# ChenKaiXuSan/Skiing_Analysis_PyTorch

Measured on AMD Instinct MI355X. Metric: 3D-pose frames/sec, 8-view 518px clips, higher is better.
Workload: dtype f16

## Files before the change

### include/skimi.h

```cpp
#ifndef SKIMI_H
#define SKIMI_H

#include <stddef.h>
#include <stdint.h>

#ifdef __cplusplus
extern "C" {
#endif

#define SKIMI_OK 0
#define SKIMI_ERR_ARG (-1)
#define SKIMI_ERR_HIP (-2)
#define SKIMI_ERR_STATE (-3)
#define SKIMI_ERR_WORKSPACE (-4)

#define SKIMI_F32 0
#define SKIMI_BF16 1
#define SKIMI_BF16X3_REC 2
#define SKIMI_FP8MX 3
#define SKIMI_F16 4

#define SKIMI_PREC_BF16 0
#define SKIMI_PREC_BF16X3 1
#define SKIMI_PREC_FP8 2
// ... 47 lines not shown
    int32_t force_splitk;
    int32_t splitk_scratch_zeroed;
    const void* W_split;
    void* x3_scratch;
    uint64_t x3_scratch_bytes;
    void* out_records;
} skimi_gemm_desc;

int skimi_split_planes(const float* x, int64_t ld, int64_t rows, int32_t C, void* hi, void* lo, void* stream);

int skimi_split_records(const float* x, int64_t ld, int64_t rows, int32_t C, void* records, void* stream);

int skimi_dpt_fold_pack(const float* w_T, const float* b_T, const float* w_rn, int32_t C_in, int32_t C_mid, int32_t C_out,
                        int32_t s, void* w_records, float* beta, void* stream);

int skimi_gemm(const skimi_gemm_desc* d, void* stream);

#define SKIMI_GEMM_PATH_GENERIC 1
#define SKIMI_GEMM_PATH_SPLITK_ORDERED 2
#define SKIMI_GEMM_PATH_SPLITK_ATOMIC 3
#define SKIMI_GEMM_PATH_X3DMA_WIDE 4
#define SKIMI_GEMM_PATH_X3DMA_NARROW 5
#define SKIMI_GEMM_PATH_GEMM256 6
#define SKIMI_GEMM_PATH_CONV_WIN 7
int32_t skimi_gemm_last_path(void);

int skimi_quant_mx(const void* x, int32_t dtype, int64_t ldx, int64_t rows, int32_t K, void* payload, void* scales,
                   void* stream);
int skimi_layernorm_mx(const float* x, int64_t ldx, int64_t rows, int32_t C, const float* gamma, const float* beta,
                       float eps, void* payload, void* scales, void* stream);
// ... 90 lines not shown
    float* pose_enc;
    float* pose_enc_list;
    float* depth;
    float* depth_conf;
    float* world_points;
    float* world_points_conf;
    float* track;
    float* vis;
    float* conf;
    float* tokens_last;
} skimi_vggt_outputs;

int skimi_vggt_forward(skimi_vggt*, const float* images, const float* query_points, int32_t B, int32_t S,
                       int32_t H, int32_t W, int32_t n_query, const skimi_vggt_outputs* out,
                       void* workspace, size_t workspace_bytes, void* stream);

int skimi_pose_to_cameras(const float* pose_enc, int64_t rows, int32_t H, int32_t W, float* extrinsic,
                          float* intrinsic, void* stream);
int skimi_unproject_depth(const float* depth, const float* extrinsic, const float* intrinsic,
                          float* world_points, int32_t frames, int32_t H, int32_t W, void* stream);
int skimi_triangulate_dlt(const float* K, const float* R, const float* t, const float* keypoints,
                          float* joints3d, int64_t steps, int32_t views, int32_t joints, void* stream);

int skimi_triangulate_triage(const float* K, const float* R, const float* t, const float* keypoints, const float* conf,
                             double conf_thr, double err_thresh_px, int64_t steps, int32_t views, int32_t joints,
                             float* joints3d, float* joints3d_clean, double* err, double* depth, uint8_t* keep,
                             double* view_stats, double* report, void* stream);

int skimi_triangulate_robust(const float* K, const float* R, const float* t, const float* keypoints, const float* conf,
                             double conf_thr, double inlier_px, int32_t min_inliers, int32_t refine_iters, int32_t weighted,
// ... 319 lines not shown
```

### skiing_analysis_pytorch_amd/_lib.py

```python
from __future__ import annotations

import ctypes as C
from pathlib import Path

LIB_PATH = Path(__file__).resolve().parent / "lib" / "libskimi.so"

F32, BF16 = 0, 1
F16 = 4
BF16X3_REC = 2
FP8MX = 3
PREC_BF16, PREC_BF16X3, PREC_FP8 = 0, 1, 2
PREC_F16 = 3
ACT_NONE, ACT_RELU, ACT_GELU, ACT_SILU, ACT_SIGMOID = 0, 1, 2, 3, 4
GEMM_PATH_GENERIC, GEMM_PATH_SPLITK_ORDERED, GEMM_PATH_SPLITK_ATOMIC = 1, 2, 3
GEMM_PATH_X3DMA_WIDE, GEMM_PATH_X3DMA_NARROW, GEMM_PATH_GEMM256, GEMM_PATH_CONV_WIN = 4, 5, 6, 7
VP3D_CONV, VP3D_MM, VP3D_WIN, VP3D_EXPAND_MFMA, VP3D_EXPAND_VALU = 1, 2, 3, 4, 5


class SkimiError(RuntimeError):
    pass


class GemmDesc(C.Structure):

# ... 220 lines not shown
    "skimi_track_pos_embed_sample": (C.c_int, [_vp, C.c_int64, _vp, C.c_int32, C.c_int32, C.c_int32, C.c_int32, _vp]),
    "skimi_track_input": (C.c_int, [_vp, _vp, _vp, _vp, _vp, _vp, C.c_int64, C.c_int32, C.c_int32, C.c_int64, C.c_float, _vp]),
    "skimi_track_coord_update": (C.c_int, [_vp, _vp, C.c_int64, _vp, _vp, C.c_int64, C.c_int32, C.c_int32, C.c_float, _vp]),
    "skimi_track_init": (C.c_int, [_vp, _vp, _vp, C.c_int64, C.c_int32, C.c_float, _vp]),
    "skimi_track_repeat_rows": (C.c_int, [_vp, _vp, C.c_int64, C.c_int32, C.c_int32, _vp]),
    "skimi_track_bns_to_bsn": (C.c_int, [_vp, _vp, C.c_int32, C.c_int32, C.c_int32, _vp]),
    "skimi_vggt_create": (_vp, [_vp]),
    "skimi_vggt_destroy": (None, [_vp]),
    "skimi_vggt_set_weight": (C.c_int, [_vp, C.c_char_p, _vp, C.c_int64, C.c_int32]),
    "skimi_vggt_finalize": (C.c_int, [_vp]),
    "skimi_vggt_set_pos_embed": (C.c_int, [_vp, C.c_int32, C.c_int32, _vp, C.c_int32]),
    "skimi_vggt_rope_positions": (C.c_int, [_vp, C.c_int32, C.c_int32, C.c_int32, _vp]),
    "skimi_vggt_workspace_bytes": (C.c_size_t, [_vp, C.c_int32, C.c_int32, C.c_int32, C.c_int32, C.c_int32]),
    "skimi_vggt_forward": (C.c_int, [_vp, _vp, _vp, C.c_int32, C.c_int32, C.c_int32, C.c_int32, C.c_int32, _vp,
                                     _vp, C.c_size_t, _vp]),
}

_lib = None


def exported_symbols():
    return sorted(_SIGNATURES)


def lib() -> C.CDLL:
    global _lib
    if _lib is not None:
        return _lib
    if not LIB_PATH.exists():
        raise SkimiError(
# ... 37 lines not shown
```

### skiing_analysis_pytorch_amd/csrc/api.hip

```cpp
#include <stdarg.h>

#include <mutex>
#include <vector>

#include "common.h"
#include "gemm_epilogue.h"
#include "kernels.h"
#include "track_kernels.h"
#include "vggt_kernels.h"

namespace skimi {

static thread_local char g_err[512] = "";

void set_error(const char* fmt, ...) {
    va_list ap;
    va_start(ap, fmt);
    vsnprintf(g_err, sizeof(g_err), fmt, ap);
    va_end(ap);
}

int lds_opt_in(std::atomic<unsigned>& done, const void* kernel, int bytes, const char* what) {
    int dev = 0;
    if (hipGetDevice(&dev) != hipSuccess) {
// ... 157 lines not shown
    return split_records_launch(x, (long)ld, (long)rows, C, records, (hipStream_t)stream);
}

int skimi_dpt_fold_pack(const float* w_T, const float* b_T, const float* w_rn, int32_t C_in, int32_t C_mid, int32_t C_out,
                        int32_t s, void* w_records, float* beta, void* stream) {
    SKIMI_CHECK_ARG(w_T && w_rn && w_records && beta, "skimi_dpt_fold_pack: null buffer");
    SKIMI_CHECK_ARG(s >= 2 && s <= 16 && C_in > 0 && C_in % 32 == 0 && C_mid > 0 && C_out > 0, "skimi_dpt_fold_pack: bad sizes");
    float* tmp = nullptr;
    SKIMI_HIP(hipMalloc((void**)&tmp, (size_t)(s + 2) * (s + 2) * C_out * C_in * 4));
    const int rc = dpt_fold_pack_launch(w_T, b_T, w_rn, C_in, C_mid, C_out, s, tmp, w_records, beta, (hipStream_t)stream);
    const hipError_t e = hipStreamSynchronize((hipStream_t)stream);
    (void)hipFree(tmp);
    if (rc) return rc;
    SKIMI_HIP(e);
    return SKIMI_OK;
}

int skimi_quant_mx(const void* x, int32_t dtype, int64_t ldx, int64_t rows, int32_t K, void* payload, void* scales,
                   void* stream) {
    return quant_mx_launch(x, dtype, (long)ldx, (long)rows, K, payload, scales, (hipStream_t)stream);
}

int skimi_layernorm_mx(const float* x, int64_t ldx, int64_t rows, int32_t C, const float* gamma, const float* beta,
                       float eps, void* payload, void* scales, void* stream) {
    return layernorm_mx_launch(x, ldx, rows, C, gamma, beta, eps, payload, scales, (hipStream_t)stream);
}

int skimi_gemm_fp8(const void* A, const void* A_scales, const void* W, const void* W_scales, int32_t M, int32_t N,
                   int32_t K, const float* bias, int32_t act, const float* gamma, const float* resid, int64_t ldr,
                   void* out, int32_t out_dtype, int64_t ldo, void* out_scales, void* stream) {
// ... 264 lines not shown
```

### skiing_analysis_pytorch_amd/csrc/vggt.hip

```cpp
#include <math.h>
#include <stdlib.h>
#include <string.h>

#include <map>
#include <memory>
#include <mutex>
#include <vector>

#include "kernels.h"
#include "vggt_kernels.h"
#include "vggt_model.h"

using namespace skimi;
using namespace skimi::vggt;

static int prepare(skimi_vggt* h, int F, int S, int H, int W, const ShapeTabs** out) {
    auto& entries = h->tabs[std::make_pair(H, W)];
    int largest = 0;
    for (const auto& e : entries) {
        if (e->frames >= F) {
            *out = e.get();
            return SKIMI_OK;
        }
        largest = std::max(largest, e->frames);
// ... 178 lines not shown
        }
    if (run_depth) {
        float* pts = out->depth ? out->depth : (float*)c.ar.alloc((size_t)F * H * W * 4);
        float* cf = out->depth_conf ? out->depth_conf : (float*)c.ar.alloc((size_t)F * H * W * 4);
        run_dpt(c, h->depth, sf, sg, F, P, nsp, ph, pw, C, H, W, pts, cf, 0);
    }
    if (run_point) {
        float* pts = out->world_points ? out->world_points : (float*)c.ar.alloc((size_t)F * H * W * 3 * 4);
        float* cf = out->world_points_conf ? out->world_points_conf : (float*)c.ar.alloc((size_t)F * H * W * 4);
        run_dpt(c, h->point, sf, sg, F, P, nsp, ph, pw, C, H, W, pts, cf, 1);
    }
    if (do_track) run_track(c, sf, sg, B, S, P, nsp, ph, pw, C, H, W, query, nq, out->track, out->vis, out->conf);
    return c.rc;
}

extern "C" {

skimi_vggt* skimi_vggt_create(const skimi_vggt_config* cfg) {
    if (!cfg) { set_error("skimi_vggt_create: null config"); return nullptr; }
    if (cfg->embed_dim <= 0 || cfg->num_heads <= 0 || cfg->embed_dim / cfg->num_heads != 64 ||
        cfg->embed_dim % cfg->num_heads != 0) {
        set_error("skimi_vggt_create: embed_dim / num_heads must be 64");
        return nullptr;
    }
    if (cfg->use_dino && cfg->embed_dim / cfg->dino_heads != 64) {
        set_error("skimi_vggt_create: DINOv2 head_dim must be 64");
        return nullptr;
    }
    if (cfg->patch_size <= 0 || cfg->depth <= 0 || cfg->num_register_tokens < 0) {
        set_error("skimi_vggt_create: bad sizes");
// ... 4 lines not shown
            set_error("skimi_vggt_create: dpt_layers[%d] = %d outside [0, depth)", i, cfg->dpt_layers[i]);
            return nullptr;
        }
    if (cfg->prec < SKIMI_PREC_BF16 || cfg->prec > SKIMI_PREC_F16) {
        set_error("skimi_vggt_create: prec %d is not one of SKIMI_PREC_BF16 / BF16X3 / FP8 / F16", cfg->prec);
        return nullptr;
    }
    if (cfg->head_prec != SKIMI_PREC_BF16 && cfg->head_prec != SKIMI_PREC_BF16X3 && cfg->head_prec != SKIMI_PREC_F16) {
        set_error("skimi_vggt_create: head_prec %d: the depth / point heads run in SKIMI_PREC_BF16X3 (the reference's fp32) or, as a "
                  "faster, less accurate option, on SKIMI_PREC_F16 / SKIMI_PREC_BF16 operands", cfg->head_prec);
        return nullptr;
    }
    skimi_vggt* h = new skimi_vggt();
    h->cfg = *cfg;
    h->dpt_fold = !(getenv("SKIMI_DPT_FOLD") && atoi(getenv("SKIMI_DPT_FOLD")) == 0);
    return h;
}

void skimi_vggt_destroy(skimi_vggt* h) {
    if (!h) return;
    for (auto& kv : h->raw) (void)hipFree(kv.second.first);
    for (void* p : h->owned) (void)hipFree(p);
    h->tabs.clear();
    for (auto& kv : h->dino_pos_alt) (void)hipFree(kv.second);
    delete h;
}

int skimi_vggt_set_weight(skimi_vggt* h, const char* key, const float* data, int64_t n, int32_t on_device) {
    SKIMI_CHECK_ARG(h && key && data && n > 0, "skimi_vggt_set_weight: bad arguments");
    float* d = nullptr;
// ... 112 lines not shown
        std::lock_guard<std::mutex> lk(h->prep_mu);
        if ((rc = prepare(h, B * S, S, H, W, &tabs))) return rc;
    }
    Ctx c{h, (hipStream_t)stream};
    c.tabs = tabs;
    c.ar.base = (char*)workspace;
    c.ar.cap = workspace_bytes;
    {
        Ctx dry{h, nullptr};
        dry.ar.dry = true;
        forward_impl(h, dry, images, query_points, B, S, H, W, n_query, out);
        if (dry.ar.peak > workspace_bytes) {
            set_error("skimi_vggt_forward: workspace %zu < %zu", workspace_bytes, dry.ar.peak);
            return SKIMI_ERR_WORKSPACE;
        }
    }
    return forward_impl(h, c, images, query_points, B, S, H, W, n_query, out);
}

}
```

### skiing_analysis_pytorch_amd/csrc/vggt_dpt.hip

```cpp
#include "env.h"
#include "gemm_epilogue.h"
#include "kernels.h"
#include "vggt_kernels.h"
#include "vggt_model.h"

namespace skimi {
namespace vggt {

const UvTab* find_uv(const ShapeTabs* h, int w, int hh, int C) {
    if (!h) return nullptr;
    for (const auto& t : h->uv)
        if (t.w == w && t.h == hh && t.C == C) return &t;
    return nullptr;
}

bool dpt_fused_ln(const DptW& w, int f2, int udt) {
    const bool off = !(int)env_once("SKIMI_TRACK_LN_FUSED", 1);
    return !off && w.feature_only && w.out_ln != nullptr && w.out_ln->g != nullptr && w.out_ln->b != nullptr && f2 == 128 && udt == SKIMI_F32;
}

static int uv_missing() {
    set_error("uv table missing");
    return SKIMI_ERR_STATE;
}

void* run_dpt(Ctx& c, const DptW& w, float* const* sf, float* const* sg, int F, int P, int nsp, int ph, int pw, int C,
              int H, int W, float* pts, float* conf, int act_mode) {
    const int prec = w.proj[0].prec;
    const int adt = Ctx::act_dt(prec);
    const size_t es = Ctx::esz(adt);
    const int D = 2 * C, np = ph * pw, feat = w.features;
    const size_t mk = c.ar.mark();
    int hh[4] = {ph * 4, ph * 2, ph, (ph - 1) / 2 + 1};
    int ww[4] = {pw * 4, pw * 2, pw, (pw - 1) / 2 + 1};
// ... 73 lines not shown
                c.gemm(d);
            }
            {
                auto d = c.desc(w.rn[i].lin, t1, adt, w.oc[i], F * hh[i] * ww[i], rn[i], adt, feat);
                c.conv_geom(d, w.rn[i], F, hh[i], ww[i], hh[i], ww[i]);
                d.act = SKIMI_ACT_RELU;
                d.out_records = rn_rec[i];
                c.gemm(d);
            }
            c.ar.release(mk3);
        }
        c.ar.release(mk2);
    }
    void* prev = nullptr;
    char* prev_rec = nullptr;
    for (int r = 3; r >= 0; --r) {
        const FusionW& f = w.ref[r];
        const int h0 = hh[r], w0 = ww[r];
        const int M = F * h0 * w0;
        const size_t bytes = (size_t)M * feat * es;
        const bool recs = use_rec[r];
        auto conv_in = [&](const ConvW& cw, const void* in_f32, char* in_rec, void* out_f32, char* out_rec) {
            auto d = c.desc(cw.lin, in_f32, adt, feat, M, out_f32, adt, feat);
            c.conv_geom(d, cw, F, h0, w0, h0, w0);
            if (recs) d = Ctx::as_records(d, in_rec, rec_bytes(r) - 256);
            d.out_records = out_rec;
            return d;
        };
        void* cur;
        char* cur_rec = nullptr;
// ... 14 lines not shown
            cur = rn[r];
            cur_rec = rn_rec[r];
        }
        const bool u_recs = recs && takes_records(f.out_conv, nullptr, r);
        void* u = u_recs ? nullptr : c.ar.alloc(bytes);
        char* u_rec = u_recs ? (char*)c.ar.alloc(rec_bytes(r)) : nullptr;
        {
            auto d1 = conv_in(f.r2c1, cur, cur_rec, tmp, tmp_rec);
            d1.act = SKIMI_ACT_RELU;
            c.gemm(d1);
            auto d2 = conv_in(f.r2c2, tmp, tmp_rec, u, u_rec);
            d2.resid = cur; d2.ldr = feat; d2.resid_dtype = adt;
            c.gemm(d2);
        }
        const int h1 = r > 0 ? hh[r - 1] : 2 * h0, w1 = r > 0 ? ww[r - 1] : 2 * w0;
        void* olow = c.ar.alloc(bytes);
        {
            auto d = c.desc(f.out_conv, u, adt, feat, M, olow, adt, feat);
            if (u_recs) d = Ctx::as_records(d, u_rec, rec_bytes(r) - 256);
            c.gemm(d);
        }
        if (r == 0 && adt == SKIMI_F32 && w.oc1.lin.w_split != nullptr && feat % 32 == 0) {
            const size_t rec_bytes = (size_t)F * h1 * w1 * feat * 4;
            const size_t mk_rec = c.ar.mark();
            char* rec = (char*)c.ar.alloc(rec_bytes + 256);
            auto d = Ctx::as_records(c.desc(w.oc1.lin, nullptr, adt, feat, F * h1 * w1, rec, adt, w.feature_only ? feat : feat / 2), rec,
                                     rec_bytes);
            c.conv_geom(d, w.oc1, F, h1, w1, h1, w1);
            if (gemm_x3dma_eligible(&d)) {
                prev_rec = rec;
// ... 2 lines not shown
                                                     nullptr, nullptr, 1, rec + rec_bytes);
                });
                prev = nullptr;
                hh[r] = h1; ww[r] = w1;
                continue;
            }
            c.ar.release(mk_rec);
        }
        void* o = c.ar.alloc((size_t)F * h1 * w1 * feat * es);
        c.run([&] { return bilinear_ac_launch(olow, o, adt, F, h0, w0, h1, w1, feat, c.st); });
        prev = o;
        hh[r] = h1; ww[r] = w1;
    }
    const int h1 = hh[0], w1 = ww[0];
    const int f2 = w.feature_only ? feat : feat / 2;
    void* c1 = c.ar.alloc((size_t)F * h1 * w1 * f2 * es);
    if (prev_rec != nullptr) {
        auto d = Ctx::as_records(c.desc(w.oc1.lin, nullptr, adt, feat, F * h1 * w1, c1, adt, f2), prev_rec, (size_t)F * h1 * w1 * feat * 4);
        c.conv_geom(d, w.oc1, F, h1, w1, h1, w1);
        c.gemm(d);
    } else {
        auto d = c.desc(w.oc1.lin, prev, adt, feat, F * h1 * w1, c1, adt, f2);
        c.conv_geom(d, w.oc1, F, h1, w1, h1, w1);
        c.gemm(d);
    }
    const int Ho = ph * c.h->cfg.patch_size / w.down_ratio, Wo = pw * c.h->cfg.patch_size / w.down_ratio;
    const UvTab* uvt = w.pos_embed ? find_uv(c.tabs, Wo, Ho, f2) : nullptr;
    if (w.pos_embed && !uvt) c.run(uv_missing);
    const int no_direct = !(int)env_once("SKIMI_CONV_DIRECT", 1);
    const bool direct = !w.feature_only && w.oc2a_direct != nullptr && adt == SKIMI_F32 && !no_direct;
    void* c2 = nullptr;
    if (direct) {
// ... 44 lines not shown
```

### skiing_analysis_pytorch_amd/csrc/vggt_kernels.h

```cpp
#pragma once
#include "common.h"

namespace skimi {

int patch_gather_launch(const float* img, void* out, int out_dtype, int F, int H, int W, int p, int Kp,
                        hipStream_t st);
int special_tokens_launch(float* x, const float* table, int F, int S, int P, int n, int C, hipStream_t st);
int bilinear_ac_planes_launch(const float* in, unsigned short* out, int N, int h, int w, int H, int W, int C, hipStream_t st,
                              const float* tabx = nullptr, const float* taby = nullptr,
                              int slice_records = 0, void* zpage = nullptr);
int bilinear_ac_launch(const void* in, void* out, int dtype, int N, int h, int w, int H, int W, int C,
                       hipStream_t st, const float* tabx = nullptr, const float* taby = nullptr, int out_dtype = -1,
                       const float* ln_g = nullptr, const float* ln_b = nullptr, float ln_eps = 0.f);
int add_uv_pos_launch(void* x, int dtype, const float* tabx, const float* taby, int N, int H, int W, int C,
                      hipStream_t st);
int add_uv_pos_records_launch(const float* x, const float* tabx, const float* taby, int N, int H, int W, int C, void* rec,
                              hipStream_t st);
int dpt_fold_pack_launch(const float* wT, const float* bT, const float* wrn, int Ci, int Cm, int Co, int s, float* tmp, void* rec,
                         float* beta, hipStream_t st);
int adaln_launch(const float* xn, const float* x, const float* mod, float* out, long rows, int D, hipStream_t st);
int pose_update_launch(const float* delta, float* pred_pad, float* act_out, long rows, int first, hipStream_t st);
int dpt_out_launch(const void* in, int dtype, const float* W, const float* b, int n_out, float* pts, float* conf,
                   long npix, int mode, hipStream_t st);
int f32_to_bf16_launch(const float* in, void* out, long n, hipStream_t st);
int f32_to_f16_launch(const float* in, void* out, long n, hipStream_t st);
int permute_conv_launch(const float* in, float* out, int Co, int Ci, int kh, int kw, hipStream_t st, int slice_major = 0);
int permute_convT_launch(const float* in, float* out, int Ci, int Co, int s, hipStream_t st);
int pad_cols_launch(const float* in, float* out, long rows, int K, int Kp, hipStream_t st);
int tile_vec_launch(const float* in, float* out, int n, int reps, hipStream_t st);

struct BilinearTap {
    int i0, i1;
    float l0, l1;
};
// ... 24 lines not shown
```

### skiing_analysis_pytorch_amd/csrc/vggt_kernels.hip

```cpp
#include <algorithm>

#include "common.h"
#include "gemm_epilogue.h"
#include "vggt_kernels.h"

namespace skimi {

static inline int grid_for(long n, int per_block = 256, int cap = 8192) {
    return (int)std::max<long>(1, std::min<long>(cdiv(n, per_block), cap));
}

template <typename T, bool F16 = false>
__global__ __launch_bounds__(256) void patch_gather_kernel(const float* __restrict__ img, T* __restrict__ out,
                                                           int F, int H, int W, int p, int Kp) {
    const int ph = H / p, pw = W / p, K = 3 * p * p;
    const long total = (long)F * ph * pw * Kp;
    const float mean[3] = {0.485f, 0.456f, 0.406f};
    const float stdv[3] = {0.229f, 0.224f, 0.225f};
    for (long i = (long)blockIdx.x * 256 + threadIdx.x; i < total; i += (long)gridDim.x * 256) {
        const int k = (int)(i % Kp);
        const long r = i / Kp;
        float v = 0.f;
        if (k < K) {
            const int px = (int)(r % pw);
// ... 391 lines not shown
            x = (int)((i / Ci) % kw);
            y = (int)((i / ((long)Ci * kw)) % kh);
            co = i / ((long)Ci * kw * kh);
        }
        out[i] = in[((co * Ci + ci) * kh + y) * kw + x];
    }
}
int permute_conv_launch(const float* in, float* out, int Co, int Ci, int kh, int kw, hipStream_t st, int slice_major) {
    SKIMI_CHECK_ARG(!slice_major || Ci % 32 == 0, "slice-major conv weights need Cin %% 32 == 0");
    hipLaunchKernelGGL(permute_conv_kernel, dim3(grid_for((long)Co * Ci * kh * kw)), dim3(256), 0, st, in, out, Co, Ci, kh, kw,
                       slice_major);
    SKIMI_LAUNCH_CHECK();
    return SKIMI_OK;
}

__global__ void permute_convT_kernel(const float* __restrict__ in, float* __restrict__ out, int Ci, int Co, int s) {
    const long n = (long)Ci * Co * s * s;
    for (long i = (long)blockIdx.x * 256 + threadIdx.x; i < n; i += (long)gridDim.x * 256) {
        const int ci = (int)(i % Ci);
        const long r = i / Ci;
        const int co = (int)(r % Co);
        const int ab = (int)(r / Co);
        const int a = ab / s, b = ab - a * s;
        out[i] = in[(((long)ci * Co + co) * s + a) * s + b];
    }
}
int permute_convT_launch(const float* in, float* out, int Ci, int Co, int s, hipStream_t st) {
    hipLaunchKernelGGL(permute_convT_kernel, dim3(grid_for((long)Ci * Co * s * s)), dim3(256), 0, st, in, out, Ci, Co, s);
    SKIMI_LAUNCH_CHECK();
    return SKIMI_OK;
// ... 125 lines not shown
```

### skiing_analysis_pytorch_amd/csrc/vggt_model.h

```cpp
#pragma once
#include <string.h>

#include <map>
#include <memory>
#include <mutex>
#include <string>
#include <utility>
#include <vector>

#include "common.h"

namespace skimi {
namespace vggt {

struct Lin {
    void* w = nullptr;
    int wdt = SKIMI_F32;
    float* b = nullptr;
    int N = 0, K = 0;
    int prec = SKIMI_PREC_BF16X3;
    void* w_split = nullptr;
    void* wq = nullptr;
    void* wq_scales = nullptr;
};
// ... 3 lines not shown
    Lin qkv, proj, fc1, fc2;
    float *ls1 = nullptr, *ls2 = nullptr;
    float *qn_w = nullptr, *qn_b = nullptr, *kn_w = nullptr, *kn_b = nullptr;
};
struct ConvW { Lin lin; int k = 1, stride = 1, pad = 0, cin = 0; int kmode = 1; };
struct FusionW { Lin out_conv; ConvW r1c1, r1c2, r2c1, r2c2; bool has_r1 = false; };
struct DptW {
    LNw norm;
    Lin proj[4];
    Lin rs0, rs1;
    Lin fold[2];
    ConvW rs3;
    ConvW rn[4];
    FusionW ref[4];
    ConvW oc1, oc2a;
    float *oc2b_w = nullptr, *oc2b_b = nullptr;
    unsigned short* oc2a_direct = nullptr;
    int n_out = 0, features = 0, oc[4] = {0, 0, 0, 0};
    bool feature_only = false, pos_embed = true;
    bool out_f32 = false;
    const LNw* out_ln = nullptr;
    int down_ratio = 1;
};
struct CamW {
    std::vector<BlockW> trunk;
    LNw token_norm, trunk_norm;
    float* empty16 = nullptr;
    Lin embed_pose, poseLN, fc1, fc2;
};
struct MhaW {
// ... 38 lines not shown
    std::vector<UvTab> uv;
    std::vector<void*> owned;
    ~ShapeTabs() {
        for (void* p : owned) (void)hipFree(p);
    }
};

}
}

struct skimi_vggt {
    skimi_vggt_config cfg;
    std::map<std::string, std::pair<float*, int64_t>> raw;
    std::vector<void*> owned;
    bool finalized = false;
    bool dpt_fold = true;
    skimi::vggt::Lin patch_proj;
    int patch_kp = 0;
    float* dino_pos = nullptr;
    std::map<std::pair<int, int>, float*> dino_pos_alt;
    float* dino_special = nullptr;
    float* agg_special = nullptr;
    std::vector<skimi::vggt::BlockW> dino, frame, global;
    skimi::vggt::LNw dino_norm;
    skimi::vggt::CamW cam;
    skimi::vggt::DptW depth, point, trackf;
    skimi::vggt::TrackW track;
    std::mutex prep_mu;
    std::map<std::pair<int, int>, std::vector<std::unique_ptr<skimi::vggt::ShapeTabs>>> tabs;
};
// ... 4 lines not shown
struct Packer {
    skimi_vggt* h;
    int rc = SKIMI_OK;
    hipStream_t st = nullptr;

    float* raw(const std::string& key, int64_t n);
    void* dmalloc(size_t bytes);
    float* keep(const std::string& key, int64_t n);
    LNw ln(const std::string& p, int C) { return LNw{keep(p + ".weight", C), keep(p + ".bias", C)}; }
    Lin pack_matrix(float* src, int N, int K, int prec);
    Lin linear(const std::string& p, int N, int K, int prec, bool bias = true);
    Lin linear_named(const std::string& wkey, const std::string& bkey, int N, int K, int prec);
    void add_records(Lin& L);
    ConvW conv(const std::string& p, int Co, int Ci, int k, int stride, int pad, int prec, bool bias);
    Lin convT(const std::string& p, int C, int s, int prec);
    Lin conv_fold(const std::string& pT, const std::string& pRn, int C, int Co, int s);
    void add_fp8(Lin& L, const std::string& p, int N, int K);
    BlockW block(const std::string& p, int C, int hidden, bool qk_norm, int hd, int prec_in);
    DptW dpt(const std::string& p, int D, int features, const int* oc, int n_out, bool feature_only, int prec);
};

int pack_model(skimi_vggt* h);
void pack_track(Packer& pk, skimi_vggt* h);

struct Ctx {
    skimi_vggt* h;
    hipStream_t st;
    const ShapeTabs* tabs = nullptr;
    Arena ar;
    int rc = SKIMI_OK;
// ... 20 lines not shown
    void ln(const float* x, const float* x2, long ldx, long rows, int C, const LNw& w, float eps, void* out, int odt,
            long grp_rows = 0, long grp_stride = 0, long grp_off = 0);
    void copy(void* dst, const void* src, size_t bytes);
    void zero(void* dst, size_t bytes);
};

struct BlockBufs { void* xn; void* qkv; void* ao; void* hid; void* q8 = nullptr; void* q8s = nullptr; };
struct MhaBufs { float *xn, *cn, *q, *kv, *ao, *hid; };

void run_block(Ctx& c, const BlockW& w, float* x, int batch, int seq, int C, int heads, float eps, bool rope,
               const BlockBufs& b);
void run_camera(Ctx& c, const CamW& w, const float* sf, const float* sg, int B, int S, int P, int C, float* out_list,
                float* out_last);
const UvTab* find_uv(const ShapeTabs* h, int w, int hh, int C);
bool dpt_fused_ln(const DptW& w, int f2, int udt);
void* run_dpt(Ctx& c, const DptW& w, float* const* sf, float* const* sg, int F, int P, int nsp, int ph, int pw, int C,
              int H, int W, float* pts, float* conf, int act_mode);
void run_track(Ctx& c, float* const* sf, float* const* sg, int B, int S, int P, int nsp, int ph, int pw, int C, int H, int W,
               const float* query, int N, float* out_track, float* out_vis, float* out_conf);

}
}
```

### skiing_analysis_pytorch_amd/csrc/vggt_pack.hip

```cpp
#include <stdlib.h>

#include "env.h"
#include "gemm_epilogue.h"
#include "kernels.h"
#include "vggt_kernels.h"
#include "vggt_model.h"

namespace skimi {
namespace vggt {

float* Packer::raw(const std::string& key, int64_t n) {
    if (rc) return nullptr;
    auto it = h->raw.find(key);
    if (it == h->raw.end()) {
        set_error("skimi_vggt_finalize: missing weight '%s'", key.c_str());
        rc = SKIMI_ERR_STATE;
        return nullptr;
    }
    if (it->second.second != n) {
        set_error("skimi_vggt_finalize: weight '%s' has %ld elements, expected %ld", key.c_str(),
                  (long)it->second.second, (long)n);
        rc = SKIMI_ERR_STATE;
        return nullptr;
    }
// ... 83 lines not shown
}
Lin Packer::convT(const std::string& p, int C, int s, int prec) {
    Lin L;
    float* src = raw(p + ".weight", (int64_t)C * C * s * s);
    float* bsrc = raw(p + ".bias", C);
    if (rc) return L;
    float* tmp = nullptr;
    if (hipMalloc((void**)&tmp, (size_t)C * C * s * s * 4) != hipSuccess) { rc = SKIMI_ERR_HIP; return L; }
    if ((rc = permute_convT_launch(src, tmp, C, C, s, st))) return L;
    L = pack_matrix(tmp, s * s * C, C, prec);
    if (!rc && prec == SKIMI_PREC_BF16X3 && C % 32 == 0) add_records(L);
    (void)hipStreamSynchronize(st);
    (void)hipFree(tmp);
    L.b = (float*)dmalloc((size_t)s * s * C * 4);
    if (L.b) rc = rc ? rc : tile_vec_launch(bsrc, L.b, C, s * s, st);
    return L;
}
Lin Packer::conv_fold(const std::string& pT, const std::string& pRn, int C, int Co, int s) {
    Lin L;
    L.N = Co; L.K = 4 * C; L.prec = SKIMI_PREC_BF16X3; L.wdt = SKIMI_F32;
    float* wT = raw(pT + ".weight", (int64_t)C * C * s * s);
    float* bT = raw(pT + ".bias", C);
    float* wrn = raw(pRn + ".weight", (int64_t)Co * C * 9);
    if (rc) return L;
    const size_t n = (size_t)(s + 2) * (s + 2) * Co * C;
    float* tmp = nullptr;
    if (hipMalloc((void**)&tmp, n * 4) != hipSuccess) { rc = SKIMI_ERR_HIP; return L; }
    L.w_split = dmalloc(n * 4);
    L.b = (float*)dmalloc((size_t)9 * Co * 4);
    L.w = L.w_split;
// ... 67 lines not shown
        FusionW& f = d.ref[r];
        f.out_conv = linear(rp + ".out_conv", features, features, prec);
        if (!rc && prec == SKIMI_PREC_BF16X3 && features % 32 == 0) add_records(f.out_conv);
        f.has_r1 = r != 3;
        if (f.has_r1) {
            f.r1c1 = conv(rp + ".resConfUnit1.conv1", features, features, 3, 1, 1, prec, true);
            f.r1c2 = conv(rp + ".resConfUnit1.conv2", features, features, 3, 1, 1, prec, true);
        }
        f.r2c1 = conv(rp + ".resConfUnit2.conv1", features, features, 3, 1, 1, prec, true);
        f.r2c2 = conv(rp + ".resConfUnit2.conv2", features, features, 3, 1, 1, prec, true);
    }
    if (feature_only) {
        d.oc1 = conv(p + ".scratch.output_conv1", features, features, 3, 1, 1, prec, true);
    } else {
        d.oc1 = conv(p + ".scratch.output_conv1", features / 2, features, 3, 1, 1, prec, true);
        d.oc2a = conv(p + ".scratch.output_conv2.0", 32, features / 2, 3, 1, 1, prec, true);
        if (!rc && prec == SKIMI_PREC_BF16X3 && (features / 2) % 32 == 0) {
            const int Ci = features / 2;
            float* src = raw(p + ".scratch.output_conv2.0.weight", (int64_t)32 * Ci * 9);
            d.oc2a_direct = (unsigned short*)dmalloc((size_t)32 * Ci * 9 * 2 * 2);
            if (!rc && d.oc2a_direct) rc = conv_direct_pack_launch(src, d.oc2a_direct, Ci, st);
            if (!rc && hipStreamSynchronize(st) != hipSuccess) rc = SKIMI_ERR_HIP;
        }
        d.oc2b_w = keep(p + ".scratch.output_conv2.2.weight", (int64_t)n_out * 32);
        d.oc2b_b = keep(p + ".scratch.output_conv2.2.bias", n_out);
    }
    return d;
}

int pack_model(skimi_vggt* h) {
// ... 77 lines not shown
```

### skiing_analysis_pytorch_amd/ops.py

```python
from __future__ import annotations

import ctypes as C
from typing import NamedTuple, Optional

import torch

from . import _lib
from ._lib import ACT_NONE, BF16, F16, F32, PREC_BF16, PREC_BF16X3, GemmDesc, check, lib, ptr


def _dt(t: torch.Tensor) -> int:
    if t.dtype == torch.float32:
        return F32
    if t.dtype == torch.bfloat16:
        return BF16
    if t.dtype == torch.float16:
        return F16
    raise TypeError(f"unsupported dtype {t.dtype}")


def _require_cuda(*ts):
    for t in ts:
        if t is not None and not t.is_cuda:
            raise _lib.SkimiError("libskimi ops need device (HBM) tensors; got a CPU tensor")
# ... 354 lines not shown
    d.a_mode, d.store_mode, d.ps_s, d.ps_C = 3, 2, s, Co
    d.cN, d.cH, d.cW, d.cC = F_, h, w_, Ci
    d.bias, d.act = ptr(beta), act
    d.out_dtype = _lib.F32
    if not records_only:
        if out is None:
            out = torch.empty((F_, h * s, w_ * s, Co), dtype=torch.float32, device=w_records.device)
        d.out = ptr(out)
    d.ldo = Co
    if out_records is not None:
        d.out_records = ptr(out_records)
    check(lib().skimi_gemm(C.byref(d), _lib.current_stream()), "skimi_gemm")
    return out


def split_planes(x):
    _require_cuda(x)
    rows, Cc = x.shape
    out = torch.empty((2, rows, Cc), dtype=torch.bfloat16, device=x.device)
    check(lib().skimi_split_planes(ptr(x), x.stride(0), rows, Cc, ptr(out[0]), ptr(out[1]), _lib.current_stream()),
          "skimi_split_planes")
    return out


def quant_mx(x: torch.Tensor):
    _require_cuda(x)
    x = x.contiguous()
    rows, K = x.shape
    Kp = (K + 127) // 128 * 128
    q = torch.empty((rows, Kp), dtype=torch.uint8, device=x.device)
# ... 194 lines not shown
```

Measured before the change: 18.31.

## Run DPT output_conv1 at coarse resolution via per-tap GEMM and upsample-sum kernel

For the last DPT fusion stage, the 3x3 output_conv1 is no longer applied after the 2x bilinear upsample. Instead a 9-tap weight matrix is packed so one GEMM at the coarse resolution produces per-tap outputs. A new kernel then bilinearly upsamples and sums the shifted taps with the bias, which is intended to cut conv FLOPs by about 4x and avoid materialising the upsampled map. It adds a taps buffer nine times the channel width at coarse resolution, and its boundary handling must match a zero-padded conv on the upsampled map. Arena-usage and a coarse-path counter are exposed for diagnostics.

```diff
diff --git a/include/skimi.h b/include/skimi.h
--- a/include/skimi.h
+++ b/include/skimi.h
@@ -85,6 +85,8 @@
 int skimi_dpt_fold_pack(const float* w_T, const float* b_T, const float* w_rn, int32_t C_in, int32_t C_mid, int32_t C_out,
                         int32_t s, void* w_records, float* beta, void* stream);
 
+int skimi_dpt_tap_sum(const float* taps, const float* bias, float* out, int32_t N, int32_t h, int32_t w, int32_t C, void* stream);
+
 int skimi_gemm(const skimi_gemm_desc* d, void* stream);
 
 #define SKIMI_GEMM_PATH_GENERIC 1
@@ -205,6 +207,10 @@
 int skimi_vggt_forward(skimi_vggt*, const float* images, const float* query_points, int32_t B, int32_t S,
                        int32_t H, int32_t W, int32_t n_query, const skimi_vggt_outputs* out,
                        void* workspace, size_t workspace_bytes, void* stream);
+
+int skimi_vggt_last_arena(uint64_t* planned, uint64_t* used);
+
+int32_t skimi_vggt_oc1_coarse_count(void);
 
 int skimi_pose_to_cameras(const float* pose_enc, int64_t rows, int32_t H, int32_t W, float* extrinsic,
                           float* intrinsic, void* stream);
diff --git a/skiing_analysis_pytorch_amd/_lib.py b/skiing_analysis_pytorch_amd/_lib.py
--- a/skiing_analysis_pytorch_amd/_lib.py
+++ b/skiing_analysis_pytorch_amd/_lib.py
@@ -258,6 +258,9 @@
     "skimi_vggt_workspace_bytes": (C.c_size_t, [_vp, C.c_int32, C.c_int32, C.c_int32, C.c_int32, C.c_int32]),
     "skimi_vggt_forward": (C.c_int, [_vp, _vp, _vp, C.c_int32, C.c_int32, C.c_int32, C.c_int32, C.c_int32, _vp,
                                      _vp, C.c_size_t, _vp]),
+    "skimi_vggt_last_arena": (C.c_int, [_vp, _vp]),
+    "skimi_vggt_oc1_coarse_count": (C.c_int32, []),
+    "skimi_dpt_tap_sum": (C.c_int, [_vp, _vp, _vp, C.c_int32, C.c_int32, C.c_int32, C.c_int32, _vp]),
 }
 
 _lib = None
diff --git a/skiing_analysis_pytorch_amd/csrc/api.hip b/skiing_analysis_pytorch_amd/csrc/api.hip
--- a/skiing_analysis_pytorch_amd/csrc/api.hip
+++ b/skiing_analysis_pytorch_amd/csrc/api.hip
@@ -195,6 +195,10 @@
     if (rc) return rc;
     SKIMI_HIP(e);
     return SKIMI_OK;
+}
+
+int skimi_dpt_tap_sum(const float* taps, const float* bias, float* out, int32_t N, int32_t h, int32_t w, int32_t C, void* stream) {
+    return dpt_tap_sum_launch(taps, bias, out, N, h, w, C, (hipStream_t)stream);
 }
 
 int skimi_quant_mx(const void* x, int32_t dtype, int64_t ldx, int64_t rows, int32_t K, void* payload, void* scales,
diff --git a/skiing_analysis_pytorch_amd/csrc/vggt.hip b/skiing_analysis_pytorch_amd/csrc/vggt.hip
--- a/skiing_analysis_pytorch_amd/csrc/vggt.hip
+++ b/skiing_analysis_pytorch_amd/csrc/vggt.hip
@@ -216,6 +216,8 @@
     return c.rc;
 }
 
+static thread_local size_t tl_arena_planned = 0, tl_arena_used = 0;
+
 extern "C" {
 
 skimi_vggt* skimi_vggt_create(const skimi_vggt_config* cfg) {
@@ -250,6 +252,7 @@
     skimi_vggt* h = new skimi_vggt();
     h->cfg = *cfg;
     h->dpt_fold = !(getenv("SKIMI_DPT_FOLD") && atoi(getenv("SKIMI_DPT_FOLD")) == 0);
+    h->dpt_oc1_coarse = !(getenv("SKIMI_DPT_OC1_COARSE") && atoi(getenv("SKIMI_DPT_OC1_COARSE")) == 0);
     return h;
 }
 
@@ -392,8 +395,20 @@
             set_error("skimi_vggt_forward: workspace %zu < %zu", workspace_bytes, dry.ar.peak);
             return SKIMI_ERR_WORKSPACE;
         }
-    }
-    return forward_impl(h, c, images, query_points, B, S, H, W, n_query, out);
-}
-
-}
+        tl_arena_planned = dry.ar.peak;
+    }
+    rc = forward_impl(h, c, images, query_points, B, S, H, W, n_query, out);
+    tl_arena_used = c.ar.peak;
+    return rc;
+}
+
+int skimi_vggt_last_arena(uint64_t* planned, uint64_t* used) {
+    SKIMI_CHECK_ARG(planned && used, "skimi_vggt_last_arena: null argument");
+    *planned = tl_arena_planned;
+    *used = tl_arena_used;
+    return SKIMI_OK;
+}
+
+int32_t skimi_vggt_oc1_coarse_count(void) { return dpt_oc1_coarse_count(); }
+
+}
diff --git a/skiing_analysis_pytorch_amd/csrc/vggt_dpt.hip b/skiing_analysis_pytorch_amd/csrc/vggt_dpt.hip
--- a/skiing_analysis_pytorch_amd/csrc/vggt_dpt.hip
+++ b/skiing_analysis_pytorch_amd/csrc/vggt_dpt.hip
@@ -18,6 +18,9 @@
     const bool off = !(int)env_once("SKIMI_TRACK_LN_FUSED", 1);
     return !off && w.feature_only && w.out_ln != nullptr && w.out_ln->g != nullptr && w.out_ln->b != nullptr && f2 == 128 && udt == SKIMI_F32;
 }
+
+static thread_local int tl_oc1_coarse = 0;
+int dpt_oc1_coarse_count() { return tl_oc1_coarse; }
 
 static int uv_missing() {
     set_error("uv table missing");
@@ -121,6 +124,7 @@
     }
     void* prev = nullptr;
     char* prev_rec = nullptr;
+    void* c1_coarse = nullptr;
     for (int r = 3; r >= 0; --r) {
         const FusionW& f = w.ref[r];
         const int h0 = hh[r], w0 = ww[r];
@@ -165,6 +169,28 @@
             c.gemm(d2);
         }
         const int h1 = r > 0 ? hh[r - 1] : 2 * h0, w1 = r > 0 ? ww[r - 1] : 2 * w0;
+        if (r == 0 && !w.feature_only && adt == SKIMI_F32 && w.oc1t.w_split != nullptr && feat % 32 == 0) {
+            const size_t orec_bytes = (size_t)M * feat * 4;
+            auto dt = Ctx::as_records(c.desc(w.oc1t, nullptr, adt, feat, M, fake, adt, w.oc1t.N), fake, orec_bytes);
+            if (gemm_x3dma_eligible(&dt)) {
+                c1_coarse = c.ar.alloc((size_t)F * h1 * w1 * (feat / 2) * 4);
+                const size_t mk_t = c.ar.mark();
+                char* orec = (char*)c.ar.alloc(orec_bytes + 256);
+                float* taps = (float*)c.ar.alloc((size_t)M * w.oc1t.N * 4);
+                auto d = c.desc(f.out_conv, u, adt, feat, M, nullptr, adt, feat);
+                if (u_recs) d = Ctx::as_records(d, u_rec, rec_bytes(r) - 256);
+                d.out_records = orec;
+                c.gemm(d);
+                dt = Ctx::as_records(c.desc(w.oc1t, nullptr, adt, feat, M, taps, adt, w.oc1t.N), orec, orec_bytes);
+                c.gemm(dt);
+                c.run([&] { return dpt_tap_sum_launch(taps, w.oc1.lin.b, (float*)c1_coarse, F, h0, w0, feat / 2, c.st); });
+                if (!c.dry()) ++tl_oc1_coarse;
+                c.ar.release(mk_t);
+                prev = nullptr;
+                hh[r] = h1; ww[r] = w1;
+                continue;
+            }
+        }
         void* olow = c.ar.alloc(bytes);
         {
             auto d = c.desc(f.out_conv, u, adt, feat, M, olow, adt, feat);
@@ -197,8 +223,9 @@
     }
     const int h1 = hh[0], w1 = ww[0];
     const int f2 = w.feature_only ? feat : feat / 2;
-    void* c1 = c.ar.alloc((size_t)F * h1 * w1 * f2 * es);
-    if (prev_rec != nullptr) {
+    void* c1 = c1_coarse ? c1_coarse : c.ar.alloc((size_t)F * h1 * w1 * f2 * es);
+    if (c1_coarse != nullptr) {
+    } else if (prev_rec != nullptr) {
         auto d = Ctx::as_records(c.desc(w.oc1.lin, nullptr, adt, feat, F * h1 * w1, c1, adt, f2), prev_rec, (size_t)F * h1 * w1 * feat * 4);
         c.conv_geom(d, w.oc1, F, h1, w1, h1, w1);
         c.gemm(d);
diff --git a/skiing_analysis_pytorch_amd/csrc/vggt_kernels.h b/skiing_analysis_pytorch_amd/csrc/vggt_kernels.h
--- a/skiing_analysis_pytorch_amd/csrc/vggt_kernels.h
+++ b/skiing_analysis_pytorch_amd/csrc/vggt_kernels.h
@@ -18,6 +18,8 @@
                               hipStream_t st);
 int dpt_fold_pack_launch(const float* wT, const float* bT, const float* wrn, int Ci, int Cm, int Co, int s, float* tmp, void* rec,
                          float* beta, hipStream_t st);
+int dpt_tap_sum_launch(const float* T, const float* bias, float* out, int N, int h, int w, int C, hipStream_t st);
+int permute_conv_taps_launch(const float* in, float* out, int Co, int Ci, int kh, int kw, hipStream_t st);
 int adaln_launch(const float* xn, const float* x, const float* mod, float* out, long rows, int D, hipStream_t st);
 int pose_update_launch(const float* delta, float* pred_pad, float* act_out, long rows, int first, hipStream_t st);
 int dpt_out_launch(const void* in, int dtype, const float* W, const float* b, int n_out, float* pts, float* conf,
diff --git a/skiing_analysis_pytorch_amd/csrc/vggt_kernels.hip b/skiing_analysis_pytorch_amd/csrc/vggt_kernels.hip
--- a/skiing_analysis_pytorch_amd/csrc/vggt_kernels.hip
+++ b/skiing_analysis_pytorch_amd/csrc/vggt_kernels.hip
@@ -429,6 +429,131 @@
     return SKIMI_OK;
 }
 
+__global__ void permute_conv_taps_kernel(const float* __restrict__ in, float* __restrict__ out, int Co, int Ci, int kh, int kw) {
+    const long n = (long)Co * Ci * kh * kw;
+    for (long i = (long)blockIdx.x * 256 + threadIdx.x; i < n; i += (long)gridDim.x * 256) {
+        const int ci = (int)(i % Ci);
+        const long r = i / Ci;
+        const int co = (int)(r % Co);
+        const int t = (int)(r / Co);
+        const int y = t / kw, x = t - y * kw;
+        out[i] = in[(((long)co * Ci + ci) * kh + y) * kw + x];
+    }
+}
+int permute_conv_taps_launch(const float* in, float* out, int Co, int Ci, int kh, int kw, hipStream_t st) {
+    hipLaunchKernelGGL(permute_conv_taps_kernel, dim3(grid_for((long)Co * Ci * kh * kw)), dim3(256), 0, st, in, out, Co, Ci, kh, kw);
+    SKIMI_LAUNCH_CHECK();
+    return SKIMI_OK;
+}
+
+constexpr int TS_TH = 16, TS_TW = 32;
+constexpr int TS_WR = (TS_TH + 1) / 2 + 3, TS_WC = (TS_TW + 1) / 2 + 3;
+constexpr int TS_STAGE = (TS_WR * TS_WC * 8 + 255) / 256;
+
+__global__ __launch_bounds__(256) void dpt_tap_sum_kernel(const float* __restrict__ T, const float* __restrict__ bias,
+                                                          float* __restrict__ out, int h, int w, int C) {
+#pragma clang fp contract(off)
+    __shared__ float4 win[TS_WR * TS_WC * 8];
+    const int H = 2 * h, W = 2 * w;
+    const float sy = (float)(h - 1) / (float)(H - 1), sx = (float)(w - 1) / (float)(W - 1);
+    const int X0 = blockIdx.x * TS_TW, Y0 = blockIdx.y * TS_TH;
+    const long n = blockIdx.z;
+    const int tid = threadIdx.x, c4 = tid & 7, col = tid >> 3;
+    const int ry0 = bilinear_ac_tap(sy, max(Y0 - 1, 0), h).i0, ry1 = bilinear_ac_tap(sy, min(Y0 + TS_TH, H - 1), h).i1;
+    const int cx0 = bilinear_ac_tap(sx, max(X0 - 1, 0), w).i0, cx1 = bilinear_ac_tap(sx, min(X0 + TS_TW, W - 1), w).i1;
+    const int wr = min(ry1 - ry0 + 1, TS_WR), wc = min(cx1 - cx0 + 1, TS_WC);
+    const int nwin = wr * wc * 8;
+    const int X = X0 + col;
+    const int nslice = C / 32, nstage = nslice * 9;
+    const long trow = 9L * C;
+
+    long goff[TS_STAGE];
+#pragma unroll
+    for (int k = 0; k < TS_STAGE; ++k) {
+        const int e = min(tid + k * 256, nwin - 1);
+        const int px = e >> 3, r = px / wc, cc = px - r * wc;
+        goff[k] = ((long)r * w + cc) * trow + (e & 7) * 4;
+    }
+    const float* const tbase = T + ((n * h + ry0) * (long)w + cx0) * trow;
+    static_assert(TS_STAGE == 7, "TS_EACH lists the staged float4 of a thread");
+#define TS_EACH(X) X(0) X(1) X(2) X(3) X(4) X(5) X(6)
+#define TS_DECL(k) float4 pre##k = *reinterpret_cast<const float4*>(tbase + goff[k]);
+    TS_EACH(TS_DECL)
+#undef TS_DECL
+    float4 acc[TS_TH];
+    for (int stage = 0; stage < nstage; ++stage) {
+        const int slice = stage / 9, tap = stage - slice * 9;
+        const int dy = tap / 3 - 1, dx = tap - (tap / 3) * 3 - 1;
+        if (tap == 0) {
+            const float4 b = *reinterpret_cast<const float4*>(bias + slice * 32 + c4 * 4);
+#pragma unroll
+            for (int j = 0; j < TS_TH; ++j) acc[j] = b;
+        }
+        __syncthreads();
+#define TS_PUT(k) if (tid + k * 256 < nwin) win[tid + k * 256] = pre##k;
+        TS_EACH(TS_PUT)
+#undef TS_PUT
+        __syncthreads();
+        {
+            const int nxt = min(stage + 1, nstage - 1), ns = nxt / 9;
+            const float* base = tbase + (long)(nxt - ns * 9) * C + ns * 32;
+#define TS_GET(k) pre##k = *reinterpret_cast<const float4*>(base + goff[k]);
+            TS_EACH(TS_GET)
+#undef TS_GET
+        }
+        const int Xq = X + dx;
+        const bool xin = X < W && Xq >= 0 && Xq < W;
+        const BilinearTap tx = bilinear_ac_tap(sx, min(max(Xq, 0), W - 1), w);
+        const int o0 = (tx.i0 - cx0) * 8 + c4, o1 = (tx.i1 - cx0) * 8 + c4;
+        auto hrow = [&](int i) __attribute__((always_inline)) {
+#pragma clang fp contract(off)
+            const float4 a = win[(i - ry0) * wc * 8 + o0], b = win[(i - ry0) * wc * 8 + o1];
+            return make_float4(tx.l0 * a.x + tx.l1 * b.x, tx.l0 * a.y + tx.l1 * b.y, tx.l0 * a.z + tx.l1 * b.z,
+                               tx.l0 * a.w + tx.l1 * b.w);
+        };
+        int i0 = -1, i1 = -1;
+        float4 ha = make_float4(0.f, 0.f, 0.f, 0.f), hb = ha;
+#pragma unroll
+        for (int j = 0; j < TS_TH; ++j) {
+            const int Yq = Y0 + j + dy;
+            if (Y0 + j >= H || Yq < 0 || Yq >= H) continue;
+            const BilinearTap ty = bilinear_ac_tap(sy, Yq, h);
+            if (ty.i0 != i0) {
+                ha = ty.i0 == i1 ? hb : hrow(ty.i0);
+                i0 = ty.i0;
+            }
+            if (ty.i1 != i1) {
+                hb = ty.i1 == i0 ? ha : hrow(ty.i1);
+                i1 = ty.i1;
+            }
+            if (xin) {
+                acc[j].x += ty.l0 * ha.x + ty.l1 * hb.x;
+                acc[j].y += ty.l0 * ha.y + ty.l1 * hb.y;
+                acc[j].z += ty.l0 * ha.z + ty.l1 * hb.z;
+                acc[j].w += ty.l0 * ha.w + ty.l1 * hb.w;
+            }
+        }
+        if (tap == 8 && X < W) {
+#pragma unroll
+            for (int j = 0; j < TS_TH; ++j)
+                if (Y0 + j < H) *reinterpret_cast<float4*>(out + ((n * H + Y0 + j) * (long)W + X) * C + slice * 32 + c4 * 4) = acc[j];
+        }
+    }
+}
+
+#undef TS_EACH
+
+int dpt_tap_sum_launch(const float* T, const float* bias, float* out, int N, int h, int w, int C, hipStream_t st) {
+    SKIMI_CHECK_ARG(T && bias && out, "dpt_tap_sum: null buffer");
+    SKIMI_CHECK_ARG(N > 0 && N < 65536 && h > 0 && w > 0 && h < 16384 && w < 16384 && C > 0 && C % 32 == 0,
+                    "dpt_tap_sum: needs C %% 32 == 0, N < 65536 and a coarse map below 16384 x 16384");
+    SKIMI_CHECK_ARG((((uintptr_t)T | (uintptr_t)bias | (uintptr_t)out) & 15) == 0, "dpt_tap_sum: 16-byte aligned buffers");
+    hipLaunchKernelGGL(dpt_tap_sum_kernel, dim3((unsigned)cdiv(2 * w, TS_TW), (unsigned)cdiv(2 * h, TS_TH), (unsigned)N), dim3(256), 0,
+                       st, T, bias, out, h, w, C);
+    SKIMI_LAUNCH_CHECK();
+    return SKIMI_OK;
+}
+
 __global__ void permute_convT_kernel(const float* __restrict__ in, float* __restrict__ out, int Ci, int Co, int s) {
     const long n = (long)Ci * Co * s * s;
     for (long i = (long)blockIdx.x * 256 + threadIdx.x; i < n; i += (long)gridDim.x * 256) {
diff --git a/skiing_analysis_pytorch_amd/csrc/vggt_model.h b/skiing_analysis_pytorch_amd/csrc/vggt_model.h
--- a/skiing_analysis_pytorch_amd/csrc/vggt_model.h
+++ b/skiing_analysis_pytorch_amd/csrc/vggt_model.h
@@ -41,6 +41,7 @@
     ConvW rn[4];
     FusionW ref[4];
     ConvW oc1, oc2a;
+    Lin oc1t;
     float *oc2b_w = nullptr, *oc2b_b = nullptr;
     unsigned short* oc2a_direct = nullptr;
     int n_out = 0, features = 0, oc[4] = {0, 0, 0, 0};
@@ -109,6 +110,7 @@
     std::map<std::string, std::pair<float*, int64_t>> raw;
     std::vector<void*> owned;
     bool finalized = false;
+    bool dpt_oc1_coarse = true;
     bool dpt_fold = true;
     skimi::vggt::Lin patch_proj;
     int patch_kp = 0;
@@ -143,6 +145,7 @@
     void add_records(Lin& L);
     ConvW conv(const std::string& p, int Co, int Ci, int k, int stride, int pad, int prec, bool bias);
     Lin convT(const std::string& p, int C, int s, int prec);
+    Lin conv_taps(const std::string& p, int Co, int Ci);
     Lin conv_fold(const std::string& pT, const std::string& pRn, int C, int Co, int s);
     void add_fp8(Lin& L, const std::string& p, int N, int K);
     BlockW block(const std::string& p, int C, int hidden, bool qk_norm, int hd, int prec_in);
@@ -193,6 +196,7 @@
                 float* out_last);
 const UvTab* find_uv(const ShapeTabs* h, int w, int hh, int C);
 bool dpt_fused_ln(const DptW& w, int f2, int udt);
+int dpt_oc1_coarse_count();
 void* run_dpt(Ctx& c, const DptW& w, float* const* sf, float* const* sg, int F, int P, int nsp, int ph, int pw, int C,
               int H, int W, float* pts, float* conf, int act_mode);
 void run_track(Ctx& c, float* const* sf, float* const* sg, int B, int S, int P, int nsp, int ph, int pw, int C, int H, int W,
diff --git a/skiing_analysis_pytorch_amd/csrc/vggt_pack.hip b/skiing_analysis_pytorch_amd/csrc/vggt_pack.hip
--- a/skiing_analysis_pytorch_amd/csrc/vggt_pack.hip
+++ b/skiing_analysis_pytorch_amd/csrc/vggt_pack.hip
@@ -121,6 +121,20 @@
     (void)hipFree(tmp);
     L.b = (float*)dmalloc((size_t)s * s * C * 4);
     if (L.b) rc = rc ? rc : tile_vec_launch(bsrc, L.b, C, s * s, st);
+    return L;
+}
+Lin Packer::conv_taps(const std::string& p, int Co, int Ci) {
+    Lin L;
+    float* src = raw(p + ".weight", (int64_t)Co * Ci * 9);
+    if (rc) return L;
+    float* tmp = nullptr;
+    if (hipMalloc((void**)&tmp, (size_t)9 * Co * Ci * 4) != hipSuccess) { rc = SKIMI_ERR_HIP; return L; }
+    if (!(rc = permute_conv_taps_launch(src, tmp, Co, Ci, 3, 3, st))) {
+        L = pack_matrix(tmp, 9 * Co, Ci, SKIMI_PREC_BF16X3);
+        if (!rc) add_records(L);
+    }
+    (void)hipStreamSynchronize(st);
+    (void)hipFree(tmp);
     return L;
 }
 Lin Packer::conv_fold(const std::string& pT, const std::string& pRn, int C, int Co, int s) {
@@ -218,6 +232,8 @@
         d.oc1 = conv(p + ".scratch.output_conv1", features, features, 3, 1, 1, prec, true);
     } else {
         d.oc1 = conv(p + ".scratch.output_conv1", features / 2, features, 3, 1, 1, prec, true);
+        if (h->dpt_oc1_coarse && prec == SKIMI_PREC_BF16X3 && features % 32 == 0)
+            d.oc1t = conv_taps(p + ".scratch.output_conv1", features / 2, features);
         d.oc2a = conv(p + ".scratch.output_conv2.0", 32, features / 2, 3, 1, 1, prec, true);
         if (!rc && prec == SKIMI_PREC_BF16X3 && (features / 2) % 32 == 0) {
             const int Ci = features / 2;
diff --git a/skiing_analysis_pytorch_amd/ops.py b/skiing_analysis_pytorch_amd/ops.py
--- a/skiing_analysis_pytorch_amd/ops.py
+++ b/skiing_analysis_pytorch_amd/ops.py
@@ -392,6 +392,21 @@
     return out
 
 
+def conv3x3_taps_matrix(w):
+    Co, Ci = w.shape[:2]
+    return w.permute(2, 3, 0, 1).reshape(9 * Co, Ci).contiguous()
+
+
+def dpt_tap_sum(taps, bias, *, out=None):
+    _require_cuda(taps, bias, out)
+    F_, h, w_, nine, Cc = taps.shape
+    assert nine == 9 and taps.is_contiguous() and taps.dtype == torch.float32
+    if out is None:
+        out = torch.empty((F_, 2 * h, 2 * w_, Cc), dtype=torch.float32, device=taps.device)
+    check(lib().skimi_dpt_tap_sum(ptr(taps), ptr(bias), ptr(out), F_, h, w_, Cc, _lib.current_stream()), "skimi_dpt_tap_sum")
+    return out
+
+
 def split_planes(x):
     _require_cuda(x)
     rows, Cc = x.shape
```

New measurement: 18.65, median of 6. +1.8%, better.
